# ZhangXinWhut/SimWhisper-Codec

Measured on AMD Instinct MI355X. Metric: audio-sec/sec encode+decode (RTF^-1), 16kHz batch=32x10s, higher is better.
Workload: dtype split-f16 x3 encode (f32-class, f32 accumulate) / bf16 decode (f32 accumulate); 1 GPU; batch=32x10s @16kHz per GPU (32 utterances in all), encode()+decode(), 0.1*N(0,1) seed 1234, synthetic closed-form checkpoint (291M params); precision=mixed

## Files before the change

### simwhisper_codec_amd/csrc/swc_mlp.hip

```cpp
#include <type_traits>
#include "swc_mfma.h"

namespace {

constexpr int ML_D = 768;
constexpr int ML_BM = 64;
constexpr int ML_SL = 256;
#ifndef ML_PF
#define ML_PF 16
#endif
constexpr int ML_KS1 = ML_D / 16;
constexpr int ML_KS2 = ML_SL / 16;
constexpr int ML_NB = ML_D / 4 / 32;
constexpr int ML_FPP = 96;
constexpr int ML_YP = 1040;
constexpr int ML_Y_BYTES = 2 * ML_KS1 * ML_YP;
constexpr int ML_H_BYTES = ML_SL * ML_BM * 2;
constexpr int ML_LDS = ML_Y_BYTES + ML_H_BYTES;
constexpr int ML_TLD = ML_D + 4;
static_assert(ML_KS1 * 2 == ML_FPP && ML_KS2 * ML_NB == ML_FPP, "phase length");
static_assert(ML_FPP % ML_PF == 0, "the ring index of a fragment must not depend on the phase");
static_assert(32 * ML_TLD * 4 <= ML_LDS, "epilogue buffer");
#ifndef ML_ABL
#define ML_ABL 0
#endif

template <bool F16 = false>
__device__ __forceinline__ void ml_mfma2x2_vgpr(const u32x4& a0, const u32x4& a1, const u32x4& b0, const u32x4& b1,
                                                f32x16& c00, f32x16& c01, f32x16& c10, f32x16& c11) {
    if constexpr (F16)
        asm("s_nop 1\n\t"
            "v_mfma_f32_32x32x16_f16 %0, %4, %6, %0\n\t"
            "v_mfma_f32_32x32x16_f16 %1, %4, %7, %1\n\t"
            "v_mfma_f32_32x32x16_f16 %2, %5, %6, %2\n\t"
            "v_mfma_f32_32x32x16_f16 %3, %5, %7, %3"
            : "+v"(c00), "+v"(c01), "+v"(c10), "+v"(c11)
            : "v"(a0), "v"(a1), "v"(b0), "v"(b1));
    else
        asm("s_nop 1\n\t"
            "v_mfma_f32_32x32x16_bf16 %0, %4, %6, %0\n\t"
            "v_mfma_f32_32x32x16_bf16 %1, %4, %7, %1\n\t"
            "v_mfma_f32_32x32x16_bf16 %2, %5, %6, %2\n\t"
            "v_mfma_f32_32x32x16_bf16 %3, %5, %7, %3"
            : "+v"(c00), "+v"(c01), "+v"(c10), "+v"(c11)
            : "v"(a0), "v"(a1), "v"(b0), "v"(b1));
}

__device__ __forceinline__ void ml_mfma8_1x4_vgpr(const i32x8& a, const i32x8& b0, const i32x8& b1, const i32x8& b2, const i32x8& b3,
                                                  f32x4& c0, f32x4& c1, f32x4& c2, f32x4& c3, unsigned sc) {
    asm("s_nop 1\n\t"
        "v_mfma_scale_f32_16x16x128_f8f6f4 %0, %4, %5, %0, %9, %9 op_sel_hi:[0,0,0]\n\t"
        "v_mfma_scale_f32_16x16x128_f8f6f4 %1, %4, %6, %1, %9, %9 op_sel_hi:[0,0,0]\n\t"
        "v_mfma_scale_f32_16x16x128_f8f6f4 %2, %4, %7, %2, %9, %9 op_sel_hi:[0,0,0]\n\t"
        "v_mfma_scale_f32_16x16x128_f8f6f4 %3, %4, %8, %3, %9, %9 op_sel_hi:[0,0,0]"
        : "+v"(c0), "+v"(c1), "+v"(c2), "+v"(c3)
        : "v"(a), "v"(b0), "v"(b1), "v"(b2), "v"(b3), "v"(sc));
}

template <bool F16>
__device__ __forceinline__ unsigned ml_pack_x2(float lo, float hi) {
    if constexpr (F16) {
        lo = __builtin_amdgcn_fmed3f(lo, -65504.0f, 65504.0f);
        hi = __builtin_amdgcn_fmed3f(hi, -65504.0f, 65504.0f);
        return pack_f16x2(lo, hi);
    } else {
        return pack_bf16x2(lo, hi);
    }
}

struct MlNorm {
    const float* w;
    const float* b;
};

constexpr int ML_P0 = ML_KS1 * ML_NB;
static_assert(ML_P0 % ML_PF == 0, "the ring index of a fragment must not depend on the phase");

template <bool OPROJ, bool F8 = false, bool F16 = false>
__global__ __launch_bounds__(256, 1) void mlp_block_kernel(const float* x, float* xo, MlNorm ln, float eps,
                                                           const u32x4* __restrict__ wstream, const float* __restrict__ b1,
                                                           const float* __restrict__ b2, MlNorm nln,
                                                           bf16_t* __restrict__ y_next, int M, int NS,
                                                           const bf16_t* __restrict__ att, const float* __restrict__ bo,
                                                           float alpha1, unsigned* sat) {
    static_assert(!F8 || OPROJ, "the fp8 fc1 exists for the layer-tail form");
    static_assert(!F16 || (OPROJ && !F8), "half-precision operands exist for the bf16 layer-tail form");
    constexpr int G1F = F8 ? ML_FPP / 2 : ML_FPP;
    extern __shared__ __attribute__((aligned(16))) char smem[];
    const int tid = threadIdx.x;
    const int lane = tid & 63;
    const int w = __builtin_amdgcn_readfirstlane(tid >> 6);
    const int lf = lane & 31, lh = lane >> 5;
    const int row0 = blockIdx.x * ML_BM;

    const long per_wave = (OPROJ ? ML_P0 : 0) + (long)NS * (G1F + ML_FPP) + ML_PF;
    const char* wbase = reinterpret_cast<const char*>(wstream) + (long)w * per_wave * 1024;
    const unsigned lane_off = (unsigned)lane * 16u;
    auto wfrag = [&](int i) __attribute__((always_inline)) -> u32x4 {
        if (ML_ABL & 4) i &= ML_PF - 1;
        return *reinterpret_cast<const u32x4*>(wbase + (long)i * 1024 + lane_off);
    };
    u32x4 ring[ML_PF];

    const u32x4* ylds = reinterpret_cast<const u32x4*>(smem) + lane;
    u32x4* hlds = reinterpret_cast<u32x4*>(smem + ML_Y_BYTES) + lane;
    auto y_frags = [&](int s, u32x4 (&dst)[2]) {
        if ((ML_ABL & 8) && s > 1) return;
#pragma unroll
        for (int b = 0; b < 2; ++b) dst[b] = ylds[(s * 2 + b) * (ML_YP / 16)];
    };
    f32x16 acc2[ML_NB][2];

    if constexpr (!OPROJ) {
        float4 v[16][3];
#pragma unroll
        for (int i = 0; i < 16; ++i) {
            const long row = (long)row0 + 16 * w + i;
            const bool ok = row < M && !(ML_ABL & 32);
#pragma unroll
            for (int k = 0; k < 3; ++k)
                v[i][k] = ok ? *reinterpret_cast<const float4*>(x + row * ML_D + 256 * k + 4 * lane) : make_float4(0.f, 0.f, 0.f, 0.f);
        }
        float4 gw[3], gb[3];
#pragma unroll
        for (int k = 0; k < 3; ++k) {
            gw[k] = *reinterpret_cast<const float4*>(ln.w + 256 * k + 4 * lane);
            gb[k] = *reinterpret_cast<const float4*>(ln.b + 256 * k + 4 * lane);
        }
#pragma unroll
        for (int i0 = 0; i0 < 16; i0 += 4) {
            if (i0 == 12) {
                __builtin_amdgcn_sched_barrier(0);
#pragma unroll
                for (int i = 0; i < ML_PF; ++i) ring[i] = wfrag(i);
                __builtin_amdgcn_sched_barrier(0);
            }
            float s[4], q[4], mean[4];
#pragma unroll
            for (int u = 0; u < 4; ++u) {
                s[u] = 0.f;
#pragma unroll
                for (int k = 0; k < 3; ++k) s[u] += (v[i0 + u][k].x + v[i0 + u][k].y) + (v[i0 + u][k].z + v[i0 + u][k].w);
            }
#pragma unroll
            for (int u = 0; u < 4; ++u) mean[u] = wave_sum_dpp(s[u]) / (float)ML_D;
#pragma unroll
            for (int u = 0; u < 4; ++u) {
                q[u] = 0.f;
#pragma unroll
                for (int k = 0; k < 3; ++k) {
                    const float a = v[i0 + u][k].x - mean[u], b_ = v[i0 + u][k].y - mean[u], c = v[i0 + u][k].z - mean[u],
                                d = v[i0 + u][k].w - mean[u];
                    q[u] += (a * a + b_ * b_) + (c * c + d * d);
                }
            }
#pragma unroll
            for (int u = 0; u < 4; ++u) {
                const float rstd = 1.0f / sqrtf(wave_sum_dpp(q[u]) / (float)ML_D + eps);
                const int tok = 16 * w + i0 + u;
                const int fb = tok >> 5, fl = tok & 31;
#pragma unroll
                for (int k = 0; k < 3; ++k) {
                    const float4 t = v[i0 + u][k];
                    const float o0 = (t.x - mean[u]) * rstd * gw[k].x + gb[k].x, o1 = (t.y - mean[u]) * rstd * gw[k].y + gb[k].y;
                    const float o2 = (t.z - mean[u]) * rstd * gw[k].z + gb[k].z, o3 = (t.w - mean[u]) * rstd * gw[k].w + gb[k].w;
                    const int s_ = 16 * k + (lane >> 2);
                    const int off = (s_ * 2 + fb) * ML_YP + (32 * ((lane >> 1) & 1) + fl) * 16 + (lane & 1) * 8;
                    *reinterpret_cast<uint2*>(smem + off) = make_uint2(bf16_pack2(o0, o1), bf16_pack2(o2, o3));
                }
            }
        }
        __syncthreads();
    #pragma unroll
        for (int a = 0; a < ML_NB; ++a)
#pragma unroll
            for (int b = 0; b < 2; ++b)
#pragma unroll
                for (int r = 0; r < 16; ++r) acc2[a][b][r] = 0.f;
    } else {
        const unsigned lds0 = lds_addr_of(smem);
#pragma unroll 4
        for (int i = 0; i < 2 * ML_KS1 / 4; ++i) {
            const int frag = w * (2 * ML_KS1 / 4) + i;
            const int s_ = frag >> 1, fb = frag & 1;
            int row = row0 + 32 * fb + lf;
            row = row < M ? row : M - 1;
            glds16(att + (long)row * ML_D + 16 * s_ + 8 * lh, lds0 + frag * ML_YP);
        }
#pragma unroll
        for (int n = 0; n < ML_NB; ++n) {
            if (n == ML_NB / 2) __builtin_amdgcn_sched_barrier(0);
#pragma unroll
            for (int g = 0; g < 4; ++g) {
                const int col = 192 * w + 32 * n + 8 * g + 4 * lh;
                const float4 bv = *reinterpret_cast<const float4*>(bo + col);
#pragma unroll
                for (int fb = 0; fb < 2; ++fb) {
                    const long row = (long)row0 + 32 * fb + lf;
                    const float4 xv = (row < M && !(ML_ABL & 32)) ? *reinterpret_cast<const float4*>(x + row * ML_D + col)
                                                                   : make_float4(0.f, 0.f, 0.f, 0.f);
                    acc2[n][fb][4 * g] = xv.x + bv.x; acc2[n][fb][4 * g + 1] = xv.y + bv.y;
                    acc2[n][fb][4 * g + 2] = xv.z + bv.z; acc2[n][fb][4 * g + 3] = xv.w + bv.w;
                }
            }
        }
        __builtin_amdgcn_sched_barrier(0);
#pragma unroll
        for (int i = 0; i < ML_PF; ++i) ring[i] = wfrag(i);
        asm volatile("s_waitcnt vmcnt(0)" ::: "memory");
        __syncthreads();
        if constexpr (F16) {
#pragma unroll 4
            for (int i = 0; i < 2 * ML_KS1 / 4; ++i) {
                u32x4* fp = reinterpret_cast<u32x4*>(smem + (w * (2 * ML_KS1 / 4) + i) * ML_YP) + lane;
                const u32x4 v = *fp;
                u32x4 o;
#pragma unroll
                for (int e = 0; e < 4; ++e) o[e] = ml_pack_x2<true>(__uint_as_float(v[e] << 16), __uint_as_float(v[e] & 0xffff0000u));
                *fp = o;
            }
            __syncthreads();
        }
        {
            u32x4 aA[2], aB[2];
            y_frags(0, aA);
            auto step = [&](int s_, u32x4 (&cur)[2], u32x4 (&nxt)[2]) {
                if (s_ + 1 < ML_KS1) y_frags(s_ + 1, nxt);
#pragma unroll
                for (int n = 0; n < ML_NB; ++n) {
#pragma unroll
                    for (int b = 0; b < 2; ++b) acc2[n][b] = mfma32<F16>(ring[(s_ * ML_NB + n) % ML_PF], cur[b], acc2[n][b]);
                    ring[(s_ * ML_NB + n) % ML_PF] = wfrag(s_ * ML_NB + n + ML_PF);
                }
                __builtin_amdgcn_sched_barrier(0);
            };
#pragma unroll
            for (int s_ = 0; s_ < ML_KS1; s_ += 2) {
                step(s_, aA, aB);
                step(s_ + 1, aB, aA);
            }
            wbase += ML_P0 * 1024;
        }
        float* red = reinterpret_cast<float*>(smem + ML_Y_BYTES);
        float sm[2], mean[2], rstd[2];
#pragma unroll
        for (int fb = 0; fb < 2; ++fb) {
            float t = 0.f;
#pragma unroll
            for (int n = 0; n < ML_NB; ++n)
#pragma unroll
                for (int r = 0; r < 16; r += 4) t += (acc2[n][fb][r] + acc2[n][fb][r + 1]) + (acc2[n][fb][r + 2] + acc2[n][fb][r + 3]);
            sm[fb] = t + __shfl_xor(t, 32);
        }
        if (lh == 0) { red[w * 64 + lf] = sm[0]; red[w * 64 + 32 + lf] = sm[1]; }
        __syncthreads();
#pragma unroll
        for (int fb = 0; fb < 2; ++fb) {
            const int tk = 32 * fb + lf;
            mean[fb] = ((red[tk] + red[64 + tk]) + (red[128 + tk] + red[192 + tk])) / (float)ML_D;
            float t = 0.f;
#pragma unroll
            for (int n = 0; n < ML_NB; ++n)
#pragma unroll
                for (int r = 0; r < 16; r += 4) {
                    const float a0 = acc2[n][fb][r] - mean[fb], a1 = acc2[n][fb][r + 1] - mean[fb], a2 = acc2[n][fb][r + 2] - mean[fb],
                                a3 = acc2[n][fb][r + 3] - mean[fb];
                    t += (a0 * a0 + a1 * a1) + (a2 * a2 + a3 * a3);
                }
            sm[fb] = t + __shfl_xor(t, 32);
        }
        if (lh == 0) { red[256 + w * 64 + lf] = sm[0]; red[256 + w * 64 + 32 + lf] = sm[1]; }
        __syncthreads();
#pragma unroll
        for (int fb = 0; fb < 2; ++fb) {
            const int tk = 256 + 32 * fb + lf;
            rstd[fb] = 1.0f / sqrtf(((red[tk] + red[64 + tk]) + (red[128 + tk] + red[192 + tk])) / (float)ML_D + eps);
        }
        float amax8 = 0.f;
        (void)amax8;
#pragma unroll
        for (int n = 0; n < ML_NB; ++n) {
            float4 gw[4], gb[4];
#pragma unroll
            for (int g = 0; g < 4; ++g) {
                gw[g] = *reinterpret_cast<const float4*>(ln.w + 192 * w + 32 * n + 8 * g + 4 * lh);
                gb[g] = *reinterpret_cast<const float4*>(ln.b + 192 * w + 32 * n + 8 * g + 4 * lh);
            }
#pragma unroll
            for (int fb = 0; fb < 2; ++fb)
#pragma unroll
                for (int t = 0; t < 2; ++t) {
                    float o[8];
#pragma unroll
                    for (int e = 0; e < 8; ++e) {
                        const int r = 8 * t + e;
                        o[e] = (acc2[n][fb][r] - mean[fb]) * rstd[fb] * reinterpret_cast<const float*>(&gw[r >> 2])[r & 3] +
                               reinterpret_cast<const float*>(&gb[r >> 2])[r & 3];
                    }
                    if constexpr (F8) {
                        float am = 0.f;
#pragma unroll
                        for (int hq = 0; hq < 2; ++hq) {
                            const int c = 192 * w + 32 * n + 8 * (2 * t + hq) + 4 * lh;
                            const int tok = 32 * fb + lf;
                            const int off = (((c >> 7) * 4 + (tok >> 4)) * 2 + ((c & 31) >> 4)) * 1024 +
                                            (16 * ((c & 127) >> 5) + (tok & 15)) * 16 + (c & 15);
                            *reinterpret_cast<unsigned*>(smem + off) =
                                fp8_pack4(o[4 * hq] * SWC_FP8_ACT_SCALE, o[4 * hq + 1] * SWC_FP8_ACT_SCALE, o[4 * hq + 2] * SWC_FP8_ACT_SCALE,
                                          o[4 * hq + 3] * SWC_FP8_ACT_SCALE, am);
                        }
                        if (row0 + 32 * fb + lf < M) amax8 = fmaxf(amax8, am);
                    } else {
                        if constexpr (F16)
                            *reinterpret_cast<u32x4*>(smem + (2 * (12 * w + 2 * n + t) + fb) * ML_YP + lane * 16) =
                                (u32x4){ml_pack_x2<true>(o[0], o[1]), ml_pack_x2<true>(o[2], o[3]), ml_pack_x2<true>(o[4], o[5]),
                                        ml_pack_x2<true>(o[6], o[7])};
                        else
                            *reinterpret_cast<u32x4*>(smem + (2 * (12 * w + 2 * n + t) + fb) * ML_YP + lane * 16) =
                                (u32x4){bf16_pack2(o[0], o[1]), bf16_pack2(o[2], o[3]), bf16_pack2(o[4], o[5]), bf16_pack2(o[6], o[7])};
                    }
                }
        }
        if constexpr (F8) sat_commit(sat, 1, amax8, SWC_FP8_LIMIT);
        __syncthreads();
    }
    f32x16 acc1[2][2];

    auto h_frags = [&](int q, u32x4 (&dst)[2]) {
        if ((ML_ABL & 8) && q > 1) return;
#pragma unroll
        for (int b = 0; b < 2; ++b) dst[b] = hlds[(q * 2 + b) * 64];
    };
    float4 bias_nx[2][4];
    auto load_bias = [&](int j) __attribute__((always_inline)) {
#pragma unroll
        for (int hb = 0; hb < 2; ++hb)
#pragma unroll
            for (int g = 0; g < 4; ++g)
                bias_nx[hb][g] = *reinterpret_cast<const float4*>(b1 + (long)j * ML_SL + 64 * w + 32 * hb + 8 * g + 4 * lh);
    };
    load_bias(0);
    auto gemm1 = [&](int j) __attribute__((always_inline)) {
#pragma unroll
        for (int hb = 0; hb < 2; ++hb)
#pragma unroll
            for (int b = 0; b < 2; ++b)
#pragma unroll
                for (int r = 0; r < 16; ++r) acc1[hb][b][r] = reinterpret_cast<const float*>(&bias_nx[hb][r >> 2])[r & 3];
        load_bias(j + 1 < NS ? j + 1 : 0);
        u32x4 yA[2], yB[2];
        y_frags(0, yA);
#pragma unroll
        for (int s = 0; s < ML_KS1; s += 2) {
            {
                y_frags(s + 1, yB);
                ml_mfma2x2_vgpr<F16>(ring[(2 * s) % ML_PF], ring[(2 * s + 1) % ML_PF], yA[0], yA[1], acc1[0][0], acc1[0][1], acc1[1][0],
                                acc1[1][1]);
                ring[(2 * s) % ML_PF] = wfrag(2 * s + ML_PF);
                ring[(2 * s + 1) % ML_PF] = wfrag(2 * s + 1 + ML_PF);
                __builtin_amdgcn_sched_barrier(0);
            }
            {
                y_frags((s + 2) % ML_KS1, yA);
                ml_mfma2x2_vgpr<F16>(ring[(2 * s + 2) % ML_PF], ring[(2 * s + 3) % ML_PF], yB[0], yB[1], acc1[0][0], acc1[0][1],
                                acc1[1][0], acc1[1][1]);
                ring[(2 * s + 2) % ML_PF] = wfrag(2 * s + 2 + ML_PF);
                ring[(2 * s + 3) % ML_PF] = wfrag(2 * s + 3 + ML_PF);
                __builtin_amdgcn_sched_barrier(0);
            }
        }
        asm volatile("s_nop 15\n\ts_nop 7" : "+v"(acc1[0][0]), "+v"(acc1[0][1]), "+v"(acc1[1][0]), "+v"(acc1[1][1]));
        wbase += ML_FPP * 1024;
    };
    auto gelu_half = [&](int hb, int b, int t, int h) __attribute__((always_inline)) {
        float v[4];
#pragma unroll
        for (int e = 0; e < 4; ++e) v[e] = (ML_ABL & 2) ? acc1[hb][b][8 * t + 4 * h + e] : gelu_fast(acc1[hb][b][8 * t + 4 * h + e]);
#pragma unroll
        for (int i = 0; i < 2; ++i) acc1[hb][b][4 * t + 2 * h + i] = __uint_as_float(ml_pack_x2<F16>(v[2 * i], v[2 * i + 1]));
    };
    auto store_h = [&]() __attribute__((always_inline)) {
#pragma unroll
        for (int hb = 0; hb < 2; ++hb)
#pragma unroll
            for (int b = 0; b < 2; ++b)
#pragma unroll
                for (int t = 0; t < 2; ++t)
                    hlds[((4 * w + 2 * hb + t) * 2 + b) * 64] =
                        (u32x4){__float_as_uint(acc1[hb][b][4 * t]), __float_as_uint(acc1[hb][b][4 * t + 1]),
                                __float_as_uint(acc1[hb][b][4 * t + 2]), __float_as_uint(acc1[hb][b][4 * t + 3])};
    };
    f32x4 a8[4][4];
    float4 bias8[4];
    auto gemm1_f8 = [&](int j) __attribute__((always_inline)) {
        if constexpr (F8) {
            const int g4 = lane >> 4;
#pragma unroll
            for (int ht = 0; ht < 4; ++ht) {
                bias8[ht] = *reinterpret_cast<const float4*>(b1 + (long)j * ML_SL + 64 * w + 16 * ht + 4 * g4);
#pragma unroll
                for (int tb = 0; tb < 4; ++tb) a8[ht][tb] = (f32x4){0.f, 0.f, 0.f, 0.f};
            }
            const u32x4* y8 = reinterpret_cast<const u32x4*>(smem) + lane;
            auto yfr = [&](int s_, i32x8 (&dst)[4]) {
#pragma unroll
                for (int tb = 0; tb < 4; ++tb) {
                    const u32x4 lo = y8[((s_ * 4 + tb) * 2) * 64], hi = y8[((s_ * 4 + tb) * 2 + 1) * 64];
                    dst[tb] = (i32x8){(int)lo.x, (int)lo.y, (int)lo.z, (int)lo.w, (int)hi.x, (int)hi.y, (int)hi.z, (int)hi.w};
                }
            };
            i32x8 yA[4], yB[4];
            yfr(0, yA);
            auto step8 = [&](int s_, i32x8 (&cur)[4], i32x8 (&nxt)[4]) {
                if (s_ + 1 < ML_D / 128) yfr(s_ + 1, nxt);
#pragma unroll
                for (int ht = 0; ht < 4; ++ht) {
                    const u32x4 lo = ring[(8 * s_ + 2 * ht) % ML_PF], hi = ring[(8 * s_ + 2 * ht + 1) % ML_PF];
                    const i32x8 wa = (i32x8){(int)lo.x, (int)lo.y, (int)lo.z, (int)lo.w, (int)hi.x, (int)hi.y, (int)hi.z, (int)hi.w};
                    ml_mfma8_1x4_vgpr(wa, cur[0], cur[1], cur[2], cur[3], a8[ht][0], a8[ht][1], a8[ht][2], a8[ht][3], 0x7f7f7f7fu);
                    ring[(8 * s_ + 2 * ht) % ML_PF] = wfrag(8 * s_ + 2 * ht + ML_PF);
                    ring[(8 * s_ + 2 * ht + 1) % ML_PF] = wfrag(8 * s_ + 2 * ht + 1 + ML_PF);
                }
                __builtin_amdgcn_sched_barrier(0);
            };
#pragma unroll
            for (int s_ = 0; s_ < ML_D / 128; s_ += 2) {
                step8(s_, yA, yB);
                step8(s_ + 1, yB, yA);
            }
#pragma unroll
            for (int ht = 0; ht < 4; ++ht) asm volatile("s_nop 15\n\ts_nop 7" : "+v"(a8[ht][0]), "+v"(a8[ht][1]), "+v"(a8[ht][2]), "+v"(a8[ht][3]));
            wbase += G1F * 1024;
        }
    };
    auto gelu_tile8 = [&](int q) __attribute__((always_inline)) {
        if constexpr (F8) {
            const int ht = q >> 2, tb = q & 3;
            const float* bb = reinterpret_cast<const float*>(&bias8[ht]);
            float v[4];
#pragma unroll
            for (int r = 0; r < 4; ++r) v[r] = gelu_fast(fmaf(a8[ht][tb][r], alpha1, bb[r]));
            a8[ht][tb][0] = __uint_as_float(bf16_pack2(v[0], v[1]));
            a8[ht][tb][1] = __uint_as_float(bf16_pack2(v[2], v[3]));
        }
    };
    auto store_h8 = [&]() __attribute__((always_inline)) {
        if constexpr (F8) {
            const int g4 = lane >> 4, tok = lane & 15;
#pragma unroll
            for (int ht = 0; ht < 4; ++ht)
#pragma unroll
                for (int tb = 0; tb < 4; ++tb) {
                    const int off = ((4 * w + ht) * 2 + (tb >> 1)) * 1024 + (32 * (g4 >> 1) + 16 * (tb & 1) + tok) * 16 + 8 * (g4 & 1);
                    *reinterpret_cast<uint2*>(smem + ML_Y_BYTES + off) =
                        make_uint2(__float_as_uint(a8[ht][tb][0]), __float_as_uint(a8[ht][tb][1]));
                }
        }
    };

    auto gemm2 = [&](auto with_gelu) __attribute__((always_inline)) {
        u32x4 hA[2], hB[2];
        h_frags(0, hA);
        auto step = [&](int q, u32x4 (&cur)[2], u32x4 (&nxt)[2]) {
            if (q + 1 < ML_KS2) h_frags(q + 1, nxt);
#pragma unroll
            for (int n = 0; n < ML_NB; ++n) {
#pragma unroll
                for (int b = 0; b < 2; ++b) acc2[n][b] = mfma32<F16>(ring[(q * ML_NB + n) % ML_PF], cur[b], acc2[n][b]);
                ring[(q * ML_NB + n) % ML_PF] = wfrag(q * ML_NB + n + ML_PF);
            }
            if constexpr (decltype(with_gelu)::value) {
                if constexpr (F8) gelu_tile8(q);
                else gelu_half(q >> 3, (q >> 2) & 1, (q >> 1) & 1, q & 1);
            }
            __builtin_amdgcn_sched_barrier(0);
        };
#pragma unroll
        for (int q = 0; q < ML_KS2; q += 2) {
            step(q, hA, hB);
            step(q + 1, hB, hA);
        }
        wbase += ML_FPP * 1024;
    };

    auto g1 = [&](int j) __attribute__((always_inline)) {
        if constexpr (F8) gemm1_f8(j);
        else gemm1(j);
    };
    auto sh = [&]() __attribute__((always_inline)) {
        if constexpr (F8) store_h8();
        else store_h();
    };
    g1(0);
#pragma unroll
    for (int q = 0; q < ML_KS2; ++q) {
        if constexpr (F8) gelu_tile8(q);
        else gelu_half(q >> 3, (q >> 2) & 1, (q >> 1) & 1, q & 1);
    }
    sh();
    __syncthreads();
    for (int j = 1; j < NS; ++j) {
        g1(j);
        gemm2(std::true_type{});
        if (!(ML_ABL & 1)) __syncthreads();
        sh();
        if (!(ML_ABL & 1)) __syncthreads();
    }
    gemm2(std::false_type{});
    __syncthreads();

    if (ML_ABL & 16) {
        float keep = 0.f;
#pragma unroll
        for (int a = 0; a < ML_NB; ++a)
#pragma unroll
            for (int b = 0; b < 2; ++b) keep += acc2[a][b][0] + acc2[a][b][7];
        if (keep == 12345.678f) xo[0] = keep;
        return;
    }
    float* tl = reinterpret_cast<float*>(smem);
    float4 c4[3], nw[3], nb[3];
#pragma unroll
    for (int k = 0; k < 3; ++k) {
        c4[k] = *reinterpret_cast<const float4*>(b2 + 256 * k + 4 * lane);
        if (y_next) {
            nw[k] = *reinterpret_cast<const float4*>(nln.w + 256 * k + 4 * lane);
            nb[k] = *reinterpret_cast<const float4*>(nln.b + 256 * k + 4 * lane);
        }
    }
#pragma unroll
    for (int p = 0; p < 2; ++p) {
        float4 rr[8][3];
#pragma unroll
        for (int i = 0; i < 8; ++i) {
            const long row = (long)row0 + 32 * p + 8 * w + i;
#pragma unroll
            for (int k = 0; k < 3; ++k)
                rr[i][k] = (!OPROJ && row < M) ? *reinterpret_cast<const float4*>(x + row * ML_D + 256 * k + 4 * lane)
                                                : make_float4(0.f, 0.f, 0.f, 0.f);
        }
#pragma unroll
        for (int n = 0; n < ML_NB; ++n)
#pragma unroll
            for (int g = 0; g < 4; ++g) {
                const f32x16& t = acc2[n][p];
                *reinterpret_cast<float4*>(tl + lf * ML_TLD + 32 * (ML_NB * w + n) + 8 * g + 4 * lh) =
                    make_float4(t[4 * g], t[4 * g + 1], t[4 * g + 2], t[4 * g + 3]);
            }
        __syncthreads();
#pragma unroll
        for (int i0 = 0; i0 < 8; i0 += 4) {
            float4 o[4][3];
            float s[4], q[4], mean[4];
#pragma unroll
            for (int u = 0; u < 4; ++u) {
                const int fl = 8 * w + i0 + u;
                const long row = (long)row0 + 32 * p + fl;
                s[u] = 0.f;
#pragma unroll
                for (int k = 0; k < 3; ++k) {
                    const float4 v = *reinterpret_cast<const float4*>(tl + fl * ML_TLD + 256 * k + 4 * lane);
                    float4 r = rr[i0 + u][k];
                    r.x += v.x + c4[k].x; r.y += v.y + c4[k].y; r.z += v.z + c4[k].z; r.w += v.w + c4[k].w;
                    o[u][k] = r;
                    if (row < M) *reinterpret_cast<float4*>(xo + row * ML_D + 256 * k + 4 * lane) = r;
                    s[u] += (r.x + r.y) + (r.z + r.w);
                }
            }
            if (y_next) {
#pragma unroll
                for (int u = 0; u < 4; ++u) mean[u] = wave_sum_dpp(s[u]) / (float)ML_D;
#pragma unroll
                for (int u = 0; u < 4; ++u) {
                    q[u] = 0.f;
#pragma unroll
                    for (int k = 0; k < 3; ++k) {
                        const float a = o[u][k].x - mean[u], b_ = o[u][k].y - mean[u], c = o[u][k].z - mean[u], d = o[u][k].w - mean[u];
                        q[u] += (a * a + b_ * b_) + (c * c + d * d);
                    }
                }
#pragma unroll
                for (int u = 0; u < 4; ++u) {
                    const float rstd = 1.0f / sqrtf(wave_sum_dpp(q[u]) / (float)ML_D + eps);
                    const long row = (long)row0 + 32 * p + 8 * w + i0 + u;
                    if (row < M) {
#pragma unroll
                        for (int k = 0; k < 3; ++k) {
                            const float4 t = o[u][k];
                            const float y0 = (t.x - mean[u]) * rstd * nw[k].x + nb[k].x, y1 = (t.y - mean[u]) * rstd * nw[k].y + nb[k].y;
                            const float y2 = (t.z - mean[u]) * rstd * nw[k].z + nb[k].z, y3 = (t.w - mean[u]) * rstd * nw[k].w + nb[k].w;
                            *reinterpret_cast<uint2*>(y_next + row * ML_D + 256 * k + 4 * lane) =
                                make_uint2(bf16_pack2(y0, y1), bf16_pack2(y2, y3));
                        }
                    }
                }
            }
        }
        __syncthreads();
    }
}

__global__ void mlp_pack_kernel(const bf16_t* __restrict__ wo, const void* __restrict__ w1v, const bf16_t* __restrict__ w2,
                                uint4* __restrict__ out, int NS, int f8) {
    const bf16_t* w1 = reinterpret_cast<const bf16_t*>(w1v);
    const unsigned char* w1q = reinterpret_cast<const unsigned char*>(w1v);
    const long p0 = wo ? ML_P0 : 0;
    const int g1f = f8 ? ML_FPP / 2 : ML_FPP;
    const long per_slice = g1f + ML_FPP;
    const long per_wave = p0 + (long)NS * per_slice + ML_PF;
    const long total = 4 * per_wave * 64;
    const long id = (long)blockIdx.x * blockDim.x + threadIdx.x;
    if (id >= total) return;
    const int lane = (int)(id & 63);
    const long f_all = id >> 6;
    const int w = (int)(f_all / per_wave);
    long f = f_all - (long)w * per_wave;
    const int lf = lane & 31, lh = lane >> 5;
    const long F = (long)NS * ML_SL;
    uint4 v = make_uint4(0, 0, 0, 0);
    if (f < p0) {
        const int s = (int)(f / ML_NB), n = (int)(f % ML_NB);
        v = *reinterpret_cast<const uint4*>(wo + (long)(192 * w + 32 * n + lf) * ML_D + 16 * s + 8 * lh);
    } else if (f - p0 < (long)NS * per_slice) {
        f -= p0;
        int j, i;
        bool is_g1;
        if (f < g1f) { is_g1 = true; j = 0; i = (int)f; }
        else {
            const long r = f - g1f;
            const long pair = r / per_slice, o = r % per_slice;
            if (pair < NS - 1) {
                if (o < g1f) { is_g1 = true; j = (int)pair + 1; i = (int)o; }
                else { is_g1 = false; j = (int)pair; i = (int)(o - g1f); }
            } else { is_g1 = false; j = NS - 1; i = (int)(r - (long)(NS - 1) * per_slice); }
        }
        if (is_g1 && f8) {
            const int s = i >> 3, ht = (i >> 1) & 3, h = i & 1;
            const long row = (long)j * ML_SL + 64 * w + 16 * ht + (lane & 15);
            v = *reinterpret_cast<const uint4*>(w1q + row * ML_D + 128 * s + 32 * (lane >> 4) + 16 * h);
        } else if (is_g1) {
            const int s = i >> 1, hb = i & 1;
            const long row = (long)j * ML_SL + 64 * w + 32 * hb + lf;
            if (wo) {
                const uint2 lo = *reinterpret_cast<const uint2*>(w1 + row * ML_D + 16 * s + 4 * lh);
                const uint2 hi = *reinterpret_cast<const uint2*>(w1 + row * ML_D + 16 * s + 4 * lh + 8);
                v = make_uint4(lo.x, lo.y, hi.x, hi.y);
            } else {
                v = *reinterpret_cast<const uint4*>(w1 + row * ML_D + 16 * s + 8 * lh);
            }
        } else {
            const int q = i / ML_NB, n = i % ML_NB;
            const long nrow = 192 * w + 32 * n + lf;
            if (f8) {
                v = *reinterpret_cast<const uint4*>(w2 + nrow * F + (long)j * ML_SL + 16 * q + 8 * lh);
            } else {
                const long hid = (long)j * ML_SL + 16 * q + 4 * lh;
                const uint2 lo = *reinterpret_cast<const uint2*>(w2 + nrow * F + hid);
                const uint2 hi = *reinterpret_cast<const uint2*>(w2 + nrow * F + hid + 8);
                v = make_uint4(lo.x, lo.y, hi.x, hi.y);
            }
        }
    }
    out[id] = v;
}

int ml_pack(const void* wo, const void* w1, const void* w2, void* stream_out, int32_t D, int32_t F, void* stream, const char* who,
            int f8 = 0) {
    SWC_CHECK_ARG(w1 && w2 && stream_out, "%s: null pointer", who);
    SWC_CHECK_ARG(D == ML_D && F > 0 && F % ML_SL == 0, "%s: needs D = %d and F a multiple of %d (D=%d F=%d)", who, ML_D, ML_SL, D, F);
    SWC_CHECK_ARG(aligned16(wo) && aligned16(w1) && aligned16(w2) && aligned16(stream_out), "%s: unaligned", who);
    const int NS = F / ML_SL;
    const long total = 4L * ((wo ? ML_P0 : 0) + (long)NS * ((f8 ? ML_FPP / 2 : ML_FPP) + ML_FPP) + ML_PF) * 64;
    hipLaunchKernelGGL(mlp_pack_kernel, dim3((unsigned)((total + 255) / 256)), dim3(256), 0, (hipStream_t)stream,
                       (const bf16_t*)wo, w1, (const bf16_t*)w2, (uint4*)stream_out, NS, f8);
    SWC_CHECK_LAUNCH(who);
    return SWC_OK;
}

}

extern "C" int64_t swc_mlp_stream_bytes(int32_t D, int32_t F) {
    if (D != ML_D || F <= 0 || F % ML_SL != 0) return 0;
    return 4L * ((long)(F / ML_SL) * (2 * ML_FPP) + ML_PF) * 1024;
}

extern "C" int swc_mlp_pack(const void* w1, const void* w2, void* stream_out, int32_t D, int32_t F, void* stream) {
    return ml_pack(nullptr, w1, w2, stream_out, D, F, stream, "swc_mlp_pack");
}

extern "C" int swc_mlp_block(const float* x, float* x_out, const float* ln_w, const float* ln_b, float eps,
                             const void* w_stream, const float* b1, const float* b2, const float* next_ln_w,
                             const float* next_ln_b, void* y_next, int32_t M, int32_t D, int32_t F, void* stream) {
    SWC_CHECK_ARG(x && x_out && ln_w && ln_b && w_stream && b1 && b2, "swc_mlp_block: null pointer");
    SWC_CHECK_ARG(!y_next || (next_ln_w && next_ln_b), "swc_mlp_block: y_next needs next_ln_w / next_ln_b");
    SWC_CHECK_ARG(D == ML_D && F > 0 && F % ML_SL == 0, "swc_mlp_block: needs D = %d and F a multiple of %d (D=%d F=%d)", ML_D,
                  ML_SL, D, F);
    SWC_CHECK_ARG(M >= 0, "swc_mlp_block: bad M");
    SWC_CHECK_ARG(aligned16(x) && aligned16(x_out) && aligned16(ln_w) && aligned16(ln_b) && aligned16(w_stream) && aligned16(b1) &&
                      aligned16(b2) && aligned16(next_ln_w) && aligned16(next_ln_b) && aligned16(y_next),
                  "swc_mlp_block: unaligned");
    if (M == 0) return SWC_OK;
    SWC_ENABLE_LDS((mlp_block_kernel<false, false>), ML_LDS, "swc_mlp_block");
    const unsigned grid = (unsigned)((M + ML_BM - 1) / ML_BM);
    hipLaunchKernelGGL((mlp_block_kernel<false, false>), dim3(grid), dim3(256), ML_LDS, (hipStream_t)stream, x, x_out, MlNorm{ln_w, ln_b},
                       eps, (const u32x4*)w_stream, b1, b2, MlNorm{next_ln_w, next_ln_b}, (bf16_t*)y_next, M, F / ML_SL,
                       (const bf16_t*)nullptr, (const float*)nullptr, 1.0f, (unsigned*)nullptr);
    SWC_CHECK_LAUNCH("swc_mlp_block");
    return SWC_OK;
}

extern "C" int64_t swc_layer_tail_stream_bytes(int32_t D, int32_t F, int32_t fc1_dtype) {
    if (D != ML_D || F <= 0 || F % ML_SL != 0 || (fc1_dtype != SWC_BF16 && fc1_dtype != SWC_FP8)) return 0;
    return 4L * (ML_P0 + (long)(F / ML_SL) * ((fc1_dtype == SWC_FP8 ? ML_FPP / 2 : ML_FPP) + ML_FPP) + ML_PF) * 1024;
}

extern "C" int swc_layer_tail_pack(const void* wo, const void* w1, const void* w2, void* stream_out, int32_t D, int32_t F,
                                   int32_t fc1_dtype, void* stream) {
    SWC_CHECK_ARG(wo, "swc_layer_tail_pack: null pointer");
    SWC_CHECK_ARG(fc1_dtype == SWC_BF16 || fc1_dtype == SWC_FP8, "swc_layer_tail_pack: fc1_dtype must be BF16 or FP8");
    return ml_pack(wo, w1, w2, stream_out, D, F, stream, "swc_layer_tail_pack", fc1_dtype == SWC_FP8);
}

extern "C" int swc_layer_tail(const void* attn, const float* x, float* x_out, const void* w_stream, const float* bo,
                              const float* ln_w, const float* ln_b, float eps, const float* b1, const float* b2,
                              const float* next_ln_w, const float* next_ln_b, void* y_next, int32_t M, int32_t D, int32_t F,
                              int32_t fc1_dtype, float fc1_alpha, int32_t operand_dtype, void* stream) {
    SWC_CHECK_ARG(operand_dtype == SWC_BF16 || (operand_dtype == SWC_F16 && fc1_dtype == SWC_BF16),
                  "swc_layer_tail: operand_dtype must be BF16, or F16 with a 16-bit fc1");
    SWC_CHECK_ARG(attn && x && x_out && bo && ln_w && ln_b && w_stream && b1 && b2, "swc_layer_tail: null pointer");
    SWC_CHECK_ARG(!y_next || (next_ln_w && next_ln_b), "swc_layer_tail: y_next needs next_ln_w / next_ln_b");
    SWC_CHECK_ARG(D == ML_D && F > 0 && F % ML_SL == 0, "swc_layer_tail: needs D = %d and F a multiple of %d (D=%d F=%d)", ML_D,
                  ML_SL, D, F);
    SWC_CHECK_ARG(fc1_dtype == SWC_BF16 || fc1_dtype == SWC_FP8, "swc_layer_tail: fc1_dtype must be BF16 or FP8");
    SWC_CHECK_ARG(M >= 0, "swc_layer_tail: bad M");
    SWC_CHECK_ARG(aligned16(attn) && aligned16(x) && aligned16(x_out) && aligned16(bo) && aligned16(ln_w) && aligned16(ln_b) &&
                      aligned16(w_stream) && aligned16(b1) && aligned16(b2) && aligned16(next_ln_w) && aligned16(next_ln_b) &&
                      aligned16(y_next),
                  "swc_layer_tail: unaligned");
    if (M == 0) return SWC_OK;
    const unsigned grid = (unsigned)((M + ML_BM - 1) / ML_BM);
    if (fc1_dtype == SWC_FP8) {
        SWC_ENABLE_LDS((mlp_block_kernel<true, true>), ML_LDS, "swc_layer_tail");
        hipLaunchKernelGGL((mlp_block_kernel<true, true>), dim3(grid), dim3(256), ML_LDS, (hipStream_t)stream, x, x_out,
                           MlNorm{ln_w, ln_b}, eps, (const u32x4*)w_stream, b1, b2, MlNorm{next_ln_w, next_ln_b}, (bf16_t*)y_next, M,
                           F / ML_SL, (const bf16_t*)attn, bo, fc1_alpha, swc_sat_counter());
    } else if (operand_dtype == SWC_F16) {
        SWC_ENABLE_LDS((mlp_block_kernel<true, false, true>), ML_LDS, "swc_layer_tail");
        hipLaunchKernelGGL((mlp_block_kernel<true, false, true>), dim3(grid), dim3(256), ML_LDS, (hipStream_t)stream, x, x_out,
                           MlNorm{ln_w, ln_b}, eps, (const u32x4*)w_stream, b1, b2, MlNorm{next_ln_w, next_ln_b}, (bf16_t*)y_next, M,
                           F / ML_SL, (const bf16_t*)attn, bo, 1.0f, (unsigned*)nullptr);
    } else {
        SWC_ENABLE_LDS((mlp_block_kernel<true, false>), ML_LDS, "swc_layer_tail");
        hipLaunchKernelGGL((mlp_block_kernel<true, false>), dim3(grid), dim3(256), ML_LDS, (hipStream_t)stream, x, x_out,
                           MlNorm{ln_w, ln_b}, eps, (const u32x4*)w_stream, b1, b2, MlNorm{next_ln_w, next_ln_b}, (bf16_t*)y_next, M,
                           F / ML_SL, (const bf16_t*)attn, bo, 1.0f, (unsigned*)nullptr);
    }
    SWC_CHECK_LAUNCH("swc_layer_tail");
    return SWC_OK;
}
```

Before: 16120 audio-s/s.

## Stream residual x loads through the output-projection K loop in two column groups

In the layer-tail MLP kernel, the residual x rows are no longer all loaded before the output-projection MFMA loop, where a full vmcnt(0) wait stalled the wave. The projection is split into two column groups run back to back. The residual tiles are prefetched a few at a time and folded into the accumulators during the loop: they are initialised for the second group and added for the first. The weight-stream packer reorders the projection fragments to match the grouped order, and the old path stays available behind ML_RES_EARLY. This raises register pressure and adds tight ordering constraints, which static asserts check.

Measured after the change: 16090 audio-s/s. About the same (-0.2%).

```diff
diff --git a/simwhisper_codec_amd/csrc/swc_mlp.hip b/simwhisper_codec_amd/csrc/swc_mlp.hip
--- a/simwhisper_codec_amd/csrc/swc_mlp.hip
+++ b/simwhisper_codec_amd/csrc/swc_mlp.hip
@@ -75,6 +75,18 @@
 
 constexpr int ML_P0 = ML_KS1 * ML_NB;
 static_assert(ML_P0 % ML_PF == 0, "the ring index of a fragment must not depend on the phase");
+#ifndef ML_RES_EARLY
+#define ML_RES_EARLY 0
+#endif
+constexpr int ML_NG = ML_RES_EARLY ? 1 : 2;
+constexpr int ML_GN = ML_NB / ML_NG;
+constexpr int ML_XQ = ML_NB * 2 * 4;
+#ifndef ML_XPRE
+#define ML_XPRE 24
+#endif
+static_assert(ML_NG <= 2 && ML_XPRE <= ML_XQ / 2 && 2 * (ML_XQ / 2 - 1 - ML_XPRE) < ML_KS1 - ML_XQ / 4 &&
+                  2 * (ML_XQ - 1 - ML_XPRE) < 2 * ML_KS1 - 4,
+              "every x load is requested before the k-step that consumes it");
 
 template <bool OPROJ, bool F8 = false, bool F16 = false>
 __global__ __launch_bounds__(256, 1) void mlp_block_kernel(const float* x, float* xo, MlNorm ln, float eps,
@@ -179,6 +191,14 @@
                 for (int r = 0; r < 16; ++r) acc2[a][b][r] = 0.f;
     } else {
         const unsigned lds0 = lds_addr_of(smem);
+#if !ML_RES_EARLY
+        float4 bv[ML_NB][4];
+#pragma unroll
+        for (int n = 0; n < ML_NB; ++n)
+#pragma unroll
+            for (int g = 0; g < 4; ++g) bv[n][g] = *reinterpret_cast<const float4*>(bo + 192 * w + 32 * n + 8 * g + 4 * lh);
+        __builtin_amdgcn_sched_barrier(0);
+#endif
 #pragma unroll 4
         for (int i = 0; i < 2 * ML_KS1 / 4; ++i) {
             const int frag = w * (2 * ML_KS1 / 4) + i;
@@ -187,6 +207,53 @@
             row = row < M ? row : M - 1;
             glds16(att + (long)row * ML_D + 16 * s_ + 8 * lh, lds0 + frag * ML_YP);
         }
+#if !ML_RES_EARLY
+        const float* xrow[2];
+#pragma unroll
+        for (int fb = 0; fb < 2; ++fb) {
+            long row = (long)row0 + 32 * fb + lf;
+            row = row < M ? row : M - 1;
+            xrow[fb] = x + row * ML_D + 192 * w + 4 * lh;
+        }
+        float4 xc[ML_XQ];
+        auto xload = [&](int j) __attribute__((always_inline)) {
+            const int q = j < ML_XQ / 2 ? j + ML_XQ / 2 : j - ML_XQ / 2;
+            xc[q] = (ML_ABL & 32) ? make_float4(0.f, 0.f, 0.f, 0.f)
+                                  : *reinterpret_cast<const float4*>(xrow[(q >> 2) & 1] + 32 * (q >> 3) + 8 * (q & 3));
+        };
+        auto xinit = [&](int q) __attribute__((always_inline)) {
+            f32x16& t = acc2[q >> 3][(q >> 2) & 1];
+            const int g = q & 3;
+            const float4 b = bv[q >> 3][g];
+            t[4 * g] = xc[q].x + b.x; t[4 * g + 1] = xc[q].y + b.y; t[4 * g + 2] = xc[q].z + b.z; t[4 * g + 3] = xc[q].w + b.w;
+        };
+        auto xadd_tile = [&](int i) __attribute__((always_inline)) {
+            f32x16& t = acc2[i >> 1][i & 1];
+#pragma unroll
+            for (int g = 0; g < 4; ++g) {
+                t[4 * g] += xc[4 * i + g].x; t[4 * g + 1] += xc[4 * i + g].y;
+                t[4 * g + 2] += xc[4 * i + g].z; t[4 * g + 3] += xc[4 * i + g].w;
+            }
+            asm volatile("" : "+a"(t));
+        };
+#pragma unroll
+        for (int i = 0; i < ML_PF; ++i) ring[i] = wfrag(i);
+        __builtin_amdgcn_sched_barrier(0);
+#pragma unroll
+        for (int j = 0; j < ML_XPRE; ++j) xload(j);
+        __builtin_amdgcn_sched_barrier(0);
+        asm volatile("s_waitcnt vmcnt(%0)" ::"n"((ML_ABL & 32) ? 0 : ML_XPRE) : "memory");
+        __syncthreads();
+#pragma unroll
+        for (int n = 0; n < ML_GN; ++n)
+#pragma unroll
+            for (int g = 0; g < 4; ++g)
+#pragma unroll
+                for (int fb = 0; fb < 2; ++fb) {
+                    acc2[n][fb][4 * g] = bv[n][g].x; acc2[n][fb][4 * g + 1] = bv[n][g].y;
+                    acc2[n][fb][4 * g + 2] = bv[n][g].z; acc2[n][fb][4 * g + 3] = bv[n][g].w;
+                }
+#else
 #pragma unroll
         for (int n = 0; n < ML_NB; ++n) {
             if (n == ML_NB / 2) __builtin_amdgcn_sched_barrier(0);
@@ -209,6 +276,7 @@
         for (int i = 0; i < ML_PF; ++i) ring[i] = wfrag(i);
         asm volatile("s_waitcnt vmcnt(0)" ::: "memory");
         __syncthreads();
+#endif
         if constexpr (F16) {
 #pragma unroll 4
             for (int i = 0; i < 2 * ML_KS1 / 4; ++i) {
@@ -221,6 +289,37 @@
             }
             __syncthreads();
         }
+#if !ML_RES_EARLY
+        {
+            u32x4 aA[2], aB[2];
+            y_frags(0, aA);
+            auto step = [&](int T, u32x4 (&cur)[2], u32x4 (&nxt)[2]) {
+                const int grp = T / ML_KS1;
+                if (T + 1 < ML_NG * ML_KS1) y_frags((T + 1) % ML_KS1, nxt);
+                if (T % 2 == 0 && T / 2 + ML_XPRE < ML_XQ) xload(T / 2 + ML_XPRE);
+                __builtin_amdgcn_sched_barrier(0);
+#pragma unroll
+                for (int nn = 0; nn < ML_GN; ++nn) {
+                    const int n = grp * ML_GN + nn, i = T * ML_GN + nn;
+#pragma unroll
+                    for (int b = 0; b < 2; ++b) acc2[n][b] = mfma32<F16>(ring[i % ML_PF], cur[b], acc2[n][b]);
+                    ring[i % ML_PF] = wfrag(i + ML_PF);
+                }
+                if (T >= ML_KS1 - ML_XQ / 4 && T < ML_KS1) {
+                    xinit(ML_XQ / 2 + 2 * (T - (ML_KS1 - ML_XQ / 4)));
+                    xinit(ML_XQ / 2 + 2 * (T - (ML_KS1 - ML_XQ / 4)) + 1);
+                }
+                if (T >= 2 * ML_KS1 - 4 * 2 * ML_GN && (T & 3) == 0) xadd_tile((T - (2 * ML_KS1 - 4 * 2 * ML_GN)) >> 2);
+                __builtin_amdgcn_sched_barrier(0);
+            };
+#pragma unroll
+            for (int T = 0; T < ML_NG * ML_KS1; T += 2) {
+                step(T, aA, aB);
+                step(T + 1, aB, aA);
+            }
+            wbase += ML_P0 * 1024;
+        }
+#else
         {
             u32x4 aA[2], aB[2];
             y_frags(0, aA);
@@ -241,6 +340,7 @@
             }
             wbase += ML_P0 * 1024;
         }
+#endif
         float* red = reinterpret_cast<float*>(smem + ML_Y_BYTES);
         float sm[2], mean[2], rstd[2];
 #pragma unroll
@@ -619,7 +719,8 @@
     const long F = (long)NS * ML_SL;
     uint4 v = make_uint4(0, 0, 0, 0);
     if (f < p0) {
-        const int s = (int)(f / ML_NB), n = (int)(f % ML_NB);
+        const int grp = (int)(f / (ML_KS1 * ML_GN)), fg = (int)(f % (ML_KS1 * ML_GN));
+        const int s = fg / ML_GN, n = grp * ML_GN + fg % ML_GN;
         v = *reinterpret_cast<const uint4*>(wo + (long)(192 * w + 32 * n + lf) * ML_D + 16 * s + 8 * lh);
     } else if (f - p0 < (long)NS * per_slice) {
         f -= p0;
```
